# thegedge/StereoReconstruction

Measured on AMD Instinct MI355X. Metric: Mdisparity-hypotheses/s (WxHxD), higher is better.
Workload: dtype f64; 1 GPU; C3: synthetic rectified 1920x1080 pair, 256 depth levels, GeodesicWeight r=5; TwoView WTA both directions + cross-check; one pair per GPU; width=1920, height=1080, depth_levels=256, window_radius=5, weights=geodesic, pairs_per_gpu=1, pair_seed_rank0=1592590339, pair_seed_of_rank_r=seed + 0x10000*r, parallelism=single GPU

## Files before the change

include/stereo_recon_hip.h:

```cpp
#ifndef STEREO_RECON_HIP_H
#define STEREO_RECON_HIP_H

#include <stdint.h>
#include <stddef.h>

#ifdef __cplusplus
extern "C" {
#endif

#define SRH_ABI_VERSION 5

enum {
	SRH_OK = 0,
	SRH_E_INVALID = -1,
	SRH_E_DEVICE = -2,
	SRH_E_NO_DEVICE = -3,
	SRH_E_CANCELLED = -4,
	SRH_E_UNSUPPORTED = -5
};

enum { SRH_WEIGHT_ADAPTIVE = 0, SRH_WEIGHT_GEODESIC = 1 };
enum { SRH_MAX_VIEWS = 64 };
#define SRH_MAX_VIEW_DIM 32767

// ... 34 lines not shown

typedef struct srh_stats {
	int64_t n_pixels;
	int64_t n_eval;
	int64_t n_eval_device;
	int32_t used_dense_path;
	int32_t used_fused_kernel;
	int32_t used_strip_kernel;
	int32_t band_retries;
	int64_t n_certified;
	int64_t n_flagged;
	int64_t band_budget_bytes;
	int64_t mvs_waves_staged, mvs_waves_listed;
	int64_t scan_tiles_template, scan_tiles_walked;
	int64_t scan_tiles_bound;
} srh_stats;

typedef struct srh_context srh_context;

typedef void (*srh_progress_fn)(int step, const char *stage, void *user);

int         srh_abi_version(void);
const char *srh_build_id(void);
const char *srh_last_error(void);
int         srh_device_count(int *count);
int         srh_hw_queues_requested(void);

void srh_params_twoview_defaults(srh_params *p);
void srh_params_mvs_defaults(srh_params *p);
int  srh_camera_from_krt(const double K[9], const double R[9], const double t[3],
// ... 260 lines not shown
```

stereoreconstruction_amd/capi.py:

```python
import ctypes as C
import os

import numpy as np

_HERE = os.path.dirname(os.path.abspath(__file__))
LIB_PATH = os.environ.get("SRH_LIBRARY") or os.path.join(_HERE, "libstereo_recon_hip.so")

SRH_OK = 0
SRH_E_INVALID, SRH_E_DEVICE, SRH_E_NO_DEVICE, SRH_E_CANCELLED, SRH_E_UNSUPPORTED = -1, -2, -3, -4, -5
WEIGHT_ADAPTIVE, WEIGHT_GEODESIC = 0, 1
MAX_VIEWS = 64
MAX_VIEW_DIM = 32767

c_double_p = C.POINTER(C.c_double)
c_int32_p = C.POINTER(C.c_int32)
c_uint8_p = C.POINTER(C.c_uint8)


class Camera(C.Structure):
    _fields_ = [
        ("K", C.c_double * 9), ("Kinv", C.c_double * 9), ("R", C.c_double * 9), ("Rinv", C.c_double * 9),
        ("t", C.c_double * 3), ("C", C.c_double * 3),
        ("dist", C.c_double * 5),
        ("is_distorted", C.c_int32), ("is_refractive", C.c_int32),
# ... 47 lines not shown


LABEL_PIXEL_NONE = -2147483648

ARITH_EXACT, ARITH_FMA, ARITH_F32, ARITH_CERTIFIED = 0, 1, 2, 3
ARITH_DEFAULT = ARITH_CERTIFIED


class Stats(C.Structure):
    _fields_ = [("n_pixels", C.c_int64), ("n_eval", C.c_int64), ("n_eval_device", C.c_int64),
                ("used_dense_path", C.c_int32), ("used_fused_kernel", C.c_int32),
                ("used_strip_kernel", C.c_int32), ("band_retries", C.c_int32),
                ("n_certified", C.c_int64), ("n_flagged", C.c_int64), ("band_budget_bytes", C.c_int64),
                ("mvs_waves_staged", C.c_int64), ("mvs_waves_listed", C.c_int64),
                ("scan_tiles_template", C.c_int64), ("scan_tiles_walked", C.c_int64),
                ("scan_tiles_bound", C.c_int64)]


class FilterInfo(C.Structure):
    _fields_ = [("holes", C.c_int64), ("gap_filled", C.c_int64), ("median_filled", C.c_int64), ("replayed", C.c_int64)]


FILTER_GAPS, FILTER_MEDIAN = 1, 2


class FuseParams(C.Structure):
    _fields_ = [("dist_threshold", C.c_double), ("normal_depth_gap", C.c_double), ("min_views", C.c_int32), ("flags", C.c_int32)]


class FuseInfo(C.Structure):
    _fields_ = [("n_points", C.c_int64), ("n_candidates", C.c_int64), ("n_claimed", C.c_int64),
# ... 949 lines not shown
        sl = np.ascontiguousarray(view_slots, dtype=np.int32)
        _check(lib().srh_comm_allgather_views(self._h, sl.ctypes.data_as(c_int32_p), len(sl)))

    def comm_destroy(self):
        _check(lib().srh_comm_destroy(self._h))

    def stats(self):
        s = Stats()
        _check(lib().srh_get_stats(self._h, C.byref(s)))
        return dict(n_pixels=s.n_pixels, n_eval=s.n_eval, n_eval_device=s.n_eval_device,
                    used_dense_path=bool(s.used_dense_path), used_fused_kernel=bool(s.used_fused_kernel),
                    used_strip_kernel=bool(s.used_strip_kernel), band_retries=s.band_retries,
                    n_certified=s.n_certified, n_flagged=s.n_flagged, band_budget_bytes=s.band_budget_bytes,
                    mvs_waves_staged=s.mvs_waves_staged, mvs_waves_listed=s.mvs_waves_listed,
                    scan_tiles_template=s.scan_tiles_template, scan_tiles_walked=s.scan_tiles_walked,
                    scan_tiles_bound=s.scan_tiles_bound)

    def profile_enable(self, on=True):
        _check(lib().srh_profile_enable(self._h, int(on)))

    def profile_reset(self):
        _check(lib().srh_profile_reset(self._h))

    def profile(self):
        buf = C.create_string_buffer(1 << 16)
        _check(lib().srh_profile_dump(self._h, buf, len(buf)))
        out = {}
        for line in buf.value.decode().splitlines():
            name, ms, n = line.split()
            out[name] = (float(ms), int(n))
        return out
# ... 1 lines not shown
```

stereoreconstruction_amd/csrc/srh_api.hip:

```cpp
#include "srh_internal.hpp"
#include "srh_subpixel.hpp"
#include "srh_mvs_subpixel.hpp"
#include "srh_geom.hpp"
#include "srh_walk.hpp"
#include "srh_speckle.hpp"
#include "srh_rectify.hpp"

#include <algorithm>
#include <cassert>
#include <cstdarg>
#include <cstdio>
#include <cstdlib>
#include <cstring>
#include <map>
#include <mutex>
#include <string>
#include <utility>
#include <limits>
#include <vector>

using namespace srh;

static thread_local char g_err[512] = "";

// ... 213 lines not shown
#ifndef SRH_MVS_SLOTS
#define SRH_MVS_SLOTS 2
#endif
struct MvsSlot {
	hipStream_t stream = nullptr;
	hipEvent_t ev = nullptr, done = nullptr;
	int *h_maxc = nullptr;
	bool own_buffers = false;
	Scratch mem;
	bool pending = false;
	int view = -1, nneigh = 0, y0 = 0, y1 = 0, cmax = 0;
	int32_t neigh[SRH_MAX_NEIGH] = {0};
	srh_params p;
};

struct srh_context {
	int device = 0;
	hipStream_t own_stream = nullptr;
	hipStream_t stream = nullptr;
	ViewHost views[SRH_MAX_VIEWS];
	DevBuf<ViewDev> d_views;
	DevBuf<int32_t> d_slots;
	int32_t slots_host[SRH_MAX_VIEWS] = {0}; int slots_n = 0;
	Scratch mem;
	hipStream_t mrf_stream[SRH_MAX_VIEWS] = { nullptr };
	hipEvent_t views_go = nullptr;
	void *mrf_host = nullptr;
	DevBuf<double> mrf_peaks;
	DevBuf<double> mvs_subpx;
	int mvs_subpx_search = 0;
	double *mvsgm_host = nullptr;
	LabelStage mrf   { "single-view MRF", "MRF", 'K' };
	LabelStage mvsgm { "single-view SGM", "SGM", 'K' };
	LabelStage tvmrf { "TwoView MRF", "TwoView MRF", 'L' };
	LabelStage tvsgm { "TwoView SGM", "TwoView SGM", 'L' };
	LabelStage *const label_stages[4] = { &mrf, &mvsgm, &tvmrf, &tvsgm };
	int geodma = 1;
	int tscan_bound = 1;
	int tscan = 1;
	int strip = 1;
	int num_cus = 256;
	bool force_walk = false;
	int list_count_pass = 0;
	int list_cmax_hint = 0;
	int list_smax_hint = 0;
	int mvs_cmax_hint = 0;
	hipStream_t side_stream = nullptr;
	hipEvent_t side_go = nullptr, side_done = nullptr;
	hipEvent_t side_tpl = nullptr;
	int mvs_async = 1;
	MvsSlot mvs_slot[SRH_MVS_SLOTS];
	int mvs_turn = 0, mvs_last = -1;
	int mvs_staged = 1;
// ... 534 lines not shown
	if (!strcmp(name, "wta_outputs")) {
		if (value != 0 && value != SRH_WTA_WINNERS && value != (SRH_WTA_WINNERS | SRH_WTA_COSTS))
			return fail(SRH_E_INVALID, "wta_outputs must be 0, 1 (SRH_WTA_WINNERS) or 3 (SRH_WTA_WINNERS | SRH_WTA_COSTS): the costs are those of the kept winners");
		c->wta_outputs = (int)value; return SRH_OK;
	}
	if (!strcmp(name, "subpixel")) {
		if (value != 0 && value != 1) return fail(SRH_E_INVALID, "subpixel must be 0 or 1");
		c->subpixel = (int)value; return SRH_OK;
	}
	if (!strcmp(name, "mvs_subpixel_search")) {
		if (value != 0 && value != 1) return fail(SRH_E_INVALID, "mvs_subpixel_search must be 0 or 1");
		c->mvs_subpx_search = (int)value; return SRH_OK;
	}
	if (!strcmp(name, "tscan")) { c->tscan = value != 0; return SRH_OK; }
	if (!strcmp(name, "tscan_bound")) { c->tscan_bound = value != 0; return SRH_OK; }
	if (!strcmp(name, "geodma")) { c->geodma = value != 0; return SRH_OK; }
	if (!strcmp(name, "f32_form")) { c->f32_form = value != 0; return SRH_OK; }
	if (!strcmp(name, "rows_masked")) { c->rows_masked = (int)value; return SRH_OK; }
	if (!strcmp(name, "side_weights")) { c->side_weights = value != 0; return SRH_OK; }
	if (!strcmp(name, "debug_mvs_cmax_hint")) { c->mvs_cmax_hint = value > 0 ? (int)((value + 7) & ~7L) : 0; return SRH_OK; }
#ifdef SRH_EXPERIMENT
	if (!strcmp(name, "exp_repeat")) { exp_set((int)value, -1); return SRH_OK; }
	if (!strcmp(name, "exp_lds_pad")) { exp_set(-1, (int)value); return SRH_OK; }
	if (!strcmp(name, "exp_scan_mode")) { exp_set_scan((int)value); return SRH_OK; }
	if (!strcmp(name, "exp_walk_mode")) { exp_set_walk((int)value); return SRH_OK; }
	if (!strcmp(name, "exp_rows_mode")) { exp_set_rows((int)value); return SRH_OK; }
#endif
	return fail(SRH_E_INVALID, "unknown option '%s'", name);
}

// ... 406 lines not shown
	HIP_TRY(hipMemcpyAsync(host, dev, bytes, hipMemcpyDeviceToHost, st));
	HIP_TRY(hipStreamSynchronize(st));
	return SRH_OK;
}

static int fetch_counters(srh_context *c, const Lane &lane, int used_dense) {
	Counters h;
	int rc;
	if ((rc = read_back(lane.stream, &h, lane.mem->cnt, sizeof(h)))) return rc;
	c->stats.n_pixels = (int64_t)h.n_pixels;
	c->stats.n_eval = (int64_t)h.n_eval;
	c->stats.n_eval_device = (int64_t)h.n_eval_device;
	c->stats.scan_tiles_template = (int64_t)h.scan_tiles_template;
	c->stats.scan_tiles_walked = (int64_t)h.scan_tiles_walked;
	c->stats.scan_tiles_bound = (int64_t)h.scan_tiles_bound;
	c->stats.mvs_waves_staged = (int64_t)h.mvs_waves_staged;
	c->stats.mvs_waves_listed = (int64_t)h.mvs_waves_listed;
	c->stats.used_dense_path = used_dense;
	c->stats.used_fused_kernel = c->last_fused ? 1 : 0;
#ifdef SRH_PROFILE_PHASES
	{
		unsigned long long g[8];
		geodesic_phases_fetch(g);
		if (g[7])
			fprintf(stderr, "[srh prof] geodesic kernel: %llu waves, cycles per wave: staging %.0f  sweeps %.0f  exp %.0f  rows out %.0f  pconst: first sweep %.0f  second sweep %.0f  rest %.0f\n",
			        g[7], (double)g[0]/g[7], (double)g[1]/g[7], (double)g[2]/g[7], (double)g[4]/g[7], (double)g[5]/g[7], (double)g[6]/g[7], (double)g[3]/g[7]);
	}
	if (h.dbg_redo[4])
		fprintf(stderr, "[srh prof] redo kernel: %llu pixels, cycles per pixel (first wave): projections + mask %.0f  walk %.0f  wait for the columns %.0f  "
		        "running minimum %.0f | second wave: columns %.0f\n", h.dbg_redo[4], (double)h.dbg_redo[0]/h.dbg_redo[4], (double)h.dbg_redo[1]/h.dbg_redo[4],
// ... 694 lines not shown
}

int TvPass::run_dense(TvDense &D) const {
	int rc;
	if ((rc = dense_prepare(D))) return rc;
	const int cost_arith = c->arith == 3 ? (D.cert ? (c->cert_form == 1 ? 5 : 3) : 0) : c->arith;
	for (int by = y0; by < y1; by += (int)D.rows) {
		if (cancelled(c)) return fail(SRH_E_CANCELLED, "cancelled");
		const int nr = std::min((int)D.rows, y1 - by);
		if ((rc = dense_band_inputs(D, by, nr, cost_arith))) return rc;
		if (D.cert) HIP_TRY(hipMemsetAsync(lane.mem->band.cflag, 0, sizeof(uint32_t), lane.stream));
		if ((rc = dense_cost_pass(D, by, nr, cost_arith, false))) return rc;
		if (D.tpl_wait) { HIP_TRY(hipStreamWaitEvent(lane.stream, c->side_tpl, 0)); D.tpl_wait = false; }
		{ Scope s(c, lane.stream, "twoview_scan_kernel");
		  launch_twoview_scan(lane.stream, c->d_views, ref, oth, W, *p, by, nr, lane.mem->band.tnum, lane.mem->band.cost, D.cstride, lane.mem->cnt, lane.mem->band.prange,
		                      D.cert ? lane.mem->band.cflag : nullptr, -1, D.cert && D.strip ? lane.mem->band.pconst : nullptr, D.tscan ? lane.mem->band.stpl : nullptr, lane.mem->band.tileflag, c->num_cus, wout, c->tscan_bound); }
		if (D.cert) {
			const int cap = redo_capacity((size_t)nr*W);
			if (twoview_redo_takes(*p, D.cstride)) {
				Scope s(c, lane.stream, "twoview_redo_kernel");
				launch_twoview_redo(lane.stream, c->d_views, ref, oth, W, *p, by, lane.mem->band.tnum, lane.mem->band.wbuf, D.strip, c->views[ref].tvp,
				                    c->views[oth].tvp, lane.mem->band.cost, D.cstride, lane.mem->band.prange, lane.mem->band.cflag, cap, lane.mem->cnt, wout);
			} else {
				{ Scope s(c, lane.stream, "twoview_refill_kernel");
				  launch_twoview_refill(lane.stream, W, *p, by, lane.mem->band.prange, lane.mem->band.cflag, cap, lane.mem->band.wbuf, D.strip, c->views[ref].tvp,
				                        c->views[oth].tvp, lane.mem->band.cost, D.cstride, lane.mem->cnt); }
				Scope s(c, lane.stream, "twoview_rescan_kernel");
				launch_twoview_scan(lane.stream, c->d_views, ref, oth, W, *p, by, nr, lane.mem->band.tnum, lane.mem->band.cost, D.cstride, lane.mem->cnt, lane.mem->band.prange,
				                    lane.mem->band.cflag, cap, nullptr, nullptr, nullptr, c->num_cus, wout);
			}
		}
// ... 2130 lines not shown
```

stereoreconstruction_amd/csrc/srh_dense.hip:

```cpp
#include "srh_internal.hpp"
#include "srh_geom.hpp"
#include "srh_walk.hpp"
#include "srh_block.hpp"

#include <algorithm>
#include <type_traits>
#include <utility>

namespace srh {

__device__ __forceinline__ double color_dist_u(uint32_t a, uint32_t b) {
	const double dr = (double)((int)(a & 255u) - (int)(b & 255u));
	const double dg = (double)((int)((a >> 8) & 255u) - (int)((b >> 8) & 255u));
	const double db = (double)((int)((a >> 16) & 255u) - (int)((b >> 16) & 255u));
	return sqrt(dr*dr + dg*dg + db*db);
}

__global__ void edge_planes_kernel(const uint32_t *__restrict__ rgba, int W, int H, double *__restrict__ edges)
{
	const size_t n = (size_t)W*H;
	const double inf = __builtin_inf();
	for (size_t i = (size_t)blockIdx.x*blockDim.x + threadIdx.x; i < n; i += (size_t)gridDim.x*blockDim.x) {
		const int x = (int)(i % (size_t)W), y = (int)(i / (size_t)W);
		const uint32_t c = rgba[i];
// ... 1551 lines not shown
			x1 = x2;
		}
	}
	return good;
}

#define TS_U 8
template <bool CERT, bool WTA>
__device__ __forceinline__
bool twoview_tscan_tile(const int bid, const ViewDev *__restrict__ views, int ref, int oth, const srh_params &P,
                        int y0, int nrows, const double *__restrict__ tnum,
                        const double *__restrict__ cost, int cstride,
                        Counters *__restrict__ cnt, const PixRange *__restrict__ prange,
                        uint32_t *__restrict__ cflag, const CertBound &cb, const double *__restrict__ pexact,
                        const ScanTemplate *__restrict__ tpl, unsigned char *smask, unsigned &n_eval_acc, unsigned &n_pix_acc, unsigned &n_flag_acc,
                        int32_t *__restrict__ wout, const int use_bound, bool &by_bound)
{
	const ViewDev &L = views[ref];
	const ViewDev &Rv = views[oth];
	const int W = L.w, OW = Rv.w, OH = Rv.h;
	const int tiles_per_row = (W + SC_TW - 1)/SC_TW;
	const int tid = threadIdx.x;
	const int trow = bid / tiles_per_row;
	const int xt = (bid % tiles_per_row)*SC_TW, x = xt + tid;
	const int y = y0 + trow;
	const int D = P.num_depth_levels;
#ifdef SRH_EXPERIMENT
	if (g_exp_scan_mode == 6) return true;
#endif
	const int nS = tpl->nS, smin = tpl->smin, smax = tpl->smax;
	const bool active = x < W && L.mask[(size_t)y*W + x] == 1;
	bool good = true;
	bool verify = true;
#ifdef SRH_EXPERIMENT
	verify = g_exp_scan_mode != 3 && g_exp_scan_mode != 5;
#endif
	by_bound = false;
	if (verify) {
		bool bpass = false;
		if (active) {
			const Ray ray = cam_unproject(L.cam, (x + 0.5) / P.image_scale, (y + 0.5) / P.image_scale);
			const TsPixel pp = ts_pixel_setup(ray, L.cam, Rv.cam, P.image_scale, tpl->tabs, tpl->tmin, tpl->tmax, y);
			good = good && pp.ok;
			if (use_bound && good) bpass = ts_pixel_passes(pp, tpl->m, ts_pixel_E(pp, tpl->m, P.image_scale, (double)(x - tpl->x0)));
		}
		if (__any(active && !good)) return false;
		if (!use_bound || __any(active && !bpass)) {
			if (active) {
				const Ray ray = cam_unproject(L.cam, (x + 0.5) / P.image_scale, (y + 0.5) / P.image_scale);
				const TsPixel pp = ts_pixel_setup(ray, L.cam, Rv.cam, P.image_scale, tpl->tabs, tpl->tmin, tpl->tmax, y);
				good = tscan_verify_labels(pp.fp, pp.nd, pp.eU, pp.dyU, P.image_scale, x, D, tpl, tnum);
			}
// ... 4 lines not shown
	if (active) {
		const PixRange pr = prange[(size_t)trow*W + x];
		lo = pr.lo;
		const int hi = pr.hi;
		int wlo = x + smin, whi = x + smax;
		if (whi == -1) whi = 0;
		if (wlo < 0) wlo = 0;
		if (whi > OW - 1) whi = OW - 1;
		good = true;
		if (nS > 0 && whi >= wlo) good = lo <= wlo && hi >= whi;
		if (y < 0 || y >= OH) good = false;
	}
	if (__any(active && !good)) return false;

	const int mbase = xt + smin, mlen = nS > 0 ? SC_TW + (smax - smin) + 1 : 0;
	for (int k = tid; k < mlen; k += SC_TW) {
		const int tx = mbase + k;
		smask[k] = ((unsigned)tx < (unsigned)OW) ? Rv.mask[(size_t)y*OW + tx] : (unsigned char)0;
	}
	__syncthreads();

	unsigned n_eval = 0, n_flag = 0;
	double depth = __builtin_nan("");
	int owin = -1, orun = -1;
	if (active) {
		n_pix_acc += 1;
		const double *crow = cost + ((size_t)trow*((W + DC_TP - 1)/DC_TP) + (x/DC_TP))*(size_t)cstride*DC_TP + (x % DC_TP);
		WtaState<int, WTA> st(-1);
		bool px_sure = false;
		if (CERT && pexact) { const double *pc = pexact + ((size_t)trow*W + x)*SRH_PC; px_sure = cert_pixel_exact(cb, pc[2], pc[3]); }
		const int xm = tid - smin;
		const int xlo = x - lo;
		int nSe = nS;
#ifdef SRH_EXPERIMENT
		if (g_exp_scan_mode == 4 || g_exp_scan_mode == 5) nSe = 0;
#endif
		auto lookups = [&](auto left_c) {
			constexpr bool LEFT = decltype(left_c)::value;
			const int32_t *seq = LEFT ? tpl->S : tpl->F;
			const int nE = nSe == 0 ? 0 : (LEFT ? nS : tpl->nF);
			for (int j0 = 0; j0 < nE; j0 += TS_U) {
				int sv[TS_U], kk[TS_U], mu[TS_U];
				unsigned char mb[TS_U];
				double c[TS_U];
				{
					const int4 sa = reinterpret_cast<const int4 *>(&seq[j0])[0], sb = reinterpret_cast<const int4 *>(&seq[j0])[1];
					sv[0] = sa.x; sv[1] = sa.y; sv[2] = sa.z; sv[3] = sa.w; sv[4] = sb.x; sv[5] = sb.y; sv[6] = sb.z; sv[7] = sb.w;
				}
#pragma unroll
				for (int u = 0; u < TS_U; ++u) {
					int s;
// ... 4 lines not shown
					} else {
						s = (sv[u] << 8) >> 8;
						mu[u] = sv[u] >> 24;
					}
					sv[u] = s;
					mb[u] = smask[xm + s];
				}
#pragma unroll
				for (int u = 0; u < TS_U; ++u) {
					const bool white = j0 + u < nE && mb[u] == 1;
					n_eval += white ? (unsigned)mu[u] : 0u;
					kk[u] = white ? xlo + sv[u] : -1;
					c[u] = crow[(unsigned)(white ? kk[u] : 0)*(unsigned)DC_TP];
				}
#pragma unroll
				for (int u = 0; u < TS_U; ++u) {
					const bool on = kk[u] >= 0;
					const double cv = c[u];
					const double t = on ? cv + P.wta_margin : __builtin_inf();
					if (CERT) {
						if (__any(on && cert_step_near(t, st.minCost, cb))) {
							if (on && cert_step_doubt(cv, t, st.minCost, kk[u] == st.win, px_sure, cb, P.max_color_diff)) n_flag = 1;
						}
					}
					st.take_sum(t, cv, kk[u]);
				}
			}
		};
		if (xt + smin < 0 || !(P.wta_margin >= 0.0)) lookups(std::true_type()); else lookups(std::false_type());
		if (st.win >= 0) depth = candidate_depth(L.cam, Rv.cam, P, cam_unproject(L.cam, (x + 0.5) / P.image_scale, (y + 0.5) / P.image_scale), lo + st.win, y);
		if (st.rejected(P.second_best_factor)) depth = __builtin_inf();
		if (CERT && st.win >= 0 && cert_ratio_doubt(st.minCost, st.secondBest, P.second_best_factor, px_sure, cb, P.max_color_diff)) n_flag = 1;
		if (CERT && n_flag) cflag[1 + atomicAdd(&cflag[0], 1u)] = (uint32_t)((size_t)trow*W + x);
		if (WTA) { owin = st.win >= 0 ? lo + st.win : -1; orun = st.run >= 0 ? lo + st.run : -1; }
	}
	if (x < W) L.depth[(size_t)y*W + x] = depth;
	if (WTA && x < W) wta_store(wout, (size_t)W*L.h, (size_t)y*W + x, owin, owin >= 0 ? y : -1, orun, orun >= 0 ? y : -1);
	n_eval_acc += n_eval; n_flag_acc += n_flag;
	return true;
}

template <bool CERT, bool WTA>
__global__ __launch_bounds__(SC_TW, (CERT && WTA) ? 6 : 7)
void twoview_tscan_kernel(const ViewDev *__restrict__ views, int ref, int oth, srh_params P,
                          int y0, int nrows, const double *__restrict__ tnum,
                          const double *__restrict__ cost, int cstride,
                          Counters *__restrict__ cnt, const PixRange *__restrict__ prange,
                          uint32_t *__restrict__ cflag, CertBound cb, const double *__restrict__ pexact,
                          const ScanTemplate *__restrict__ tpl, uint32_t *__restrict__ tilelist, int32_t *__restrict__ wout, int use_bound)
{
	__shared__ unsigned char smask[SC_TW + TS_MAXSPAN + 16];
	const int W = views[ref].w;
	const int ntiles = ((W + SC_TW - 1)/SC_TW)*nrows;
	const int tid = threadIdx.x;
	const bool tok = tpl->ok != 0;
	unsigned n_eval = 0, n_pix = 0, n_flag = 0, n_tpl = 0, n_walk = 0, n_bound = 0;
	for (int bid = blockIdx.x; bid < ntiles; bid += gridDim.x) {
		bool by_bound = false;
		const bool done = tok && twoview_tscan_tile<CERT, WTA>(bid, views, ref, oth, P, y0, nrows, tnum, cost, cstride, cnt, prange, cflag, cb, pexact,
		                                                      tpl, smask, n_eval, n_pix, n_flag, wout, use_bound, by_bound);
		if (!done) { if (tid == 0) tilelist[1 + atomicAdd(&tilelist[0], 1u)] = (uint32_t)bid; ++n_walk; } else { ++n_tpl; n_bound += by_bound ? 1u : 0u; }
		__syncthreads();
	}
	if (!cnt) return;
	n_eval = wave_sum_u32(n_eval); n_pix = wave_sum_u32(n_pix); n_flag = wave_sum_u32(n_flag);
	if (tid == 0) {
		if (n_eval) atomicAdd(&cnt->n_eval, (unsigned long long)n_eval);
		if (n_pix) atomicAdd(&cnt->n_pixels, (unsigned long long)n_pix);
		if (CERT && n_pix) atomicAdd(&cnt->n_certified, (unsigned long long)n_pix);
		if (CERT && n_flag) atomicAdd(&cnt->n_flagged, (unsigned long long)n_flag);
		if (n_tpl) atomicAdd(&cnt->scan_tiles_template, (unsigned long long)n_tpl);
		if (n_walk) atomicAdd(&cnt->scan_tiles_walked, (unsigned long long)n_walk);
		if (n_bound) atomicAdd(&cnt->scan_tiles_bound, (unsigned long long)n_bound);
	}
}

#define RSW_MAXD 1024
#define RSW_MAXC 6144
#define RD_THREADS 512
#define RD_GRID 512
template <int R, bool WTA>
__global__ __launch_bounds__(RD_THREADS)
void twoview_redo_kernel(const ViewDev *__restrict__ views, int ref, int oth, srh_params P, int y0,
                         const double *__restrict__ tnum, const double *__restrict__ wbuf, int wimg,
                         const double *__restrict__ ref_tvp, const double *__restrict__ oth_tvp,
                         double *__restrict__ cost, int cstride,
                         const PixRange *__restrict__ prange, const uint32_t *__restrict__ cflag, int cap,
                         Counters *__restrict__ cnt, int32_t *__restrict__ wout)
{
	const ViewDev &L = views[ref];
	const ViewDev &Rv = views[oth];
	const int W = L.w, OW = Rv.w, OH = Rv.h;
	const int tid = threadIdx.x;
	__shared__ double sx[RSW_MAXD], sy[RSW_MAXD];
	__shared__ unsigned short scol[RSW_MAXC];
	__shared__ double srow[4096];
	__shared__ unsigned char smask[4096 + 64];
	__shared__ int s_n;
	const uint32_t nflag = cflag[0];
	if (blockIdx.x == 0 && tid == 0 && nflag > (uint32_t)cap) atomicAdd(&cnt->cert_overflow, 1ull);
	unsigned n_cols = 0;
#ifdef SRH_PROFILE_PHASES
	unsigned long long rph[6] = {0, 0, 0, 0, 0, 0}, rt = __builtin_readcyclecounter();
#define RD_STAMP(k) do { const unsigned long long tn_ = __builtin_readcyclecounter(); rph[k] += tn_ - rt; rt = tn_; } while (0)
#else
#define RD_STAMP(k)
#endif
	for (uint32_t f = blockIdx.x; f < nflag && f < (uint32_t)cap; f += gridDim.x) {
		const uint32_t q = cflag[1 + f];
		const int x = (int)(q % (uint32_t)W), trow = (int)(q / (uint32_t)W), y = y0 + trow;
		const PixRange pr = prange[q];
		const int lo = pr.lo, hi = pr.hi;
// ... 3 lines not shown
		const bool walk = !(fabs(nd) < 1e-10);
		if (walk) {
			const SharedDivisor nd_sd = shared_divisor(nd);
			for (int d = tid; d < P.num_depth_levels; d += RD_THREADS) {
				double x2, y2;
				const bool ok = pinhole_project_label_sd(ray, nd_sd, tnum[d], Rv.cam, P.image_scale, x2, y2);
				sx[d] = ok ? x2 : __builtin_nan("");
				sy[d] = ok ? y2 : 0.0;
			}
		}
		const int span = hi >= lo ? hi - lo + 1 : 0;
		for (int k = tid; k < span && k < 4096; k += RD_THREADS) smask[k] = (y >= 0 && y < OH) ? Rv.mask[(size_t)y*OW + lo + k] : 0;
		__syncthreads();
		RD_STAMP(0);
		double *crow = cost + ((size_t)trow*((W + DC_TP - 1)/DC_TP) + (x/DC_TP))*(size_t)cstride*DC_TP + (x % DC_TP);
		if (tid == 0) {
			int n = 0;
			bool over = false;
			if (walk) {
				double x1 = __builtin_nan(""), y1 = __builtin_nan("");
				for (int d = 0; d < P.num_depth_levels && !over; ++d) {
					const double x2 = sx[d], y2 = sy[d];
					if (isnan_d(x2)) continue;
					if (isnan_d(x1)) { x1 = x2; y1 = y2; continue; }
					const double dx = x2 - x1, dy = y2 - y1;
					if (!(dx*dx + dy*dy >= 1)) continue;
					const int ix0 = trunc_sat(x1), iy0 = trunc_sat(y1), ix1 = trunc_sat(x2), iy1 = trunc_sat(y2);
					const int a = ix0 < ix1 ? ix0 : ix1, b = ix0 < ix1 ? ix1 : ix0;
					if (iy0 == y && iy1 == y && a >= lo && b <= hi) {
						for (int tx = a; tx <= b; ++tx) {
							const int k = tx - lo;
							const bool white = k < 4096 ? (smask[k] == 1) : (Rv.mask[(size_t)y*OW + tx] == 1);
							if (white) { if (n < RSW_MAXC) scol[n] = (unsigned short)k; else over = true; ++n; }
						}
// ... 2 lines not shown
						lw.begin(ix0, iy0, ix1, iy1, OW, OH);
						while (lw.has_next()) {
							int tx, ty;
							lw.current(tx, ty);
							if (tx >= 0 && ty >= 0 && tx < OW && ty < OH && Rv.mask[(size_t)ty*OW + tx] == 1 &&
							    ty == y && tx >= lo && tx <= hi) {
								if (n < RSW_MAXC) scol[n] = (unsigned short)(tx - lo); else over = true;
								++n;
							}
							lw.next();
						}
					}
					x1 = x2; y1 = y2;
				}
			}
			if (over) { atomicAdd(&cnt->cert_overflow, 1ull); n = RSW_MAXC; }
			s_n = n;
		} else if (tid >= 64) {
			const int SP = padded_stride(W);
			const WindowAt wa = window_at<R>(wbuf, wimg, W, trow, x);
			const double *lp = ref_tvp + (size_t)(y + SRH_PADY - R)*SP + (x + SRH_PADL - R);
			for (int c = lo + (tid - 64); c <= hi; c += RD_THREADS - 64) {
				const double *rp = oth_tvp + (size_t)(y + SRH_PADY - R)*SP + (c + SRH_PADL - R);
				const double cv = window_exact_cost<R>(wa.wq, wa.wrow, wa.wcol, lp, rp, SP, SP, P);
				crow[(size_t)(c - lo)*DC_TP] = cv;
				if (c - lo < 4096) srow[c - lo] = cv;
				++n_cols;
			}
		}
		RD_STAMP(1);
		__syncthreads();
		RD_STAMP(2);
		if (tid == 0) {
// ... 37 lines not shown
	if (P.window_radius == 5) { if (wout) SRH_REDO(5, true); else SRH_REDO(5, false); }
	else                      { if (wout) SRH_REDO(2, true); else SRH_REDO(2, false); }
#undef SRH_REDO
	return true;
}

void launch_scan_template(hipStream_t st, const ViewDev *views, int ref, int oth, const srh_params &P, int y0, int nrows,
                          const double *tnum, void *tpl)
{
	hipLaunchKernelGGL(twoview_template_kernel, dim3(1), dim3(256), 0, st, views, ref, oth, P, y0, nrows, tnum, (ScanTemplate *)tpl);
}

void launch_twoview_scan(hipStream_t st, const ViewDev *views, int ref, int oth, int width, const srh_params &P,
                         int y0, int nrows, const double *tnum, const double *cost, int cstride,
                         Counters *cnt, const PixRange *prange, uint32_t *cflag, int nlist, const double *pexact,
                         const void *tpl, uint32_t *tilelist, int num_cus, int32_t *wout, int tscan_bound)
{
	const int tiles = (width + SC_TW - 1)/SC_TW;
	const CertBound cb = cert_bound(P);
	const ScanTemplate *tp = (const ScanTemplate *)tpl;
	if (!tp) tilelist = nullptr;
	const unsigned pgrid = (unsigned)std::min<long long>((long long)tiles*nrows, (long long)num_cus*4*8);
	const unsigned wgrid = tp ? (unsigned)std::min<long long>((long long)tiles*nrows, (long long)num_cus*4*4) : (unsigned)(tiles*nrows);
	if (tp) (void)hipMemsetAsync(tilelist, 0, sizeof(uint32_t), st);
#define SRH_TSCAN(C_, W_, FLAG_, PEX_)                                                                         \
	hipLaunchKernelGGL((twoview_tscan_kernel<C_, W_>), dim3(pgrid), dim3(SC_TW), 0, st,                        \
	                   views, ref, oth, P, y0, nrows, tnum, cost, cstride, cnt, prange, FLAG_, cb, PEX_, tp, tilelist, wout, tscan_bound)
#define SRH_SCAN(C_, L_, W_, GRID_, FLAG_, NL_, PEX_, TL_)                                                     \
	hipLaunchKernelGGL((twoview_scan_kernel<C_, L_, W_>), dim3(GRID_), dim3(SC_TW), 0, st,                     \
	                   views, ref, oth, P, y0, nrows, tnum, cost, cstride, cnt, prange, FLAG_, NL_, cb, PEX_, TL_, wout)
	if (!cflag) {
		if (tp) { if (wout) SRH_TSCAN(false, true, nullptr, nullptr); else SRH_TSCAN(false, false, nullptr, nullptr); }
		if (wout) SRH_SCAN(false, false, true, wgrid, nullptr, 0, nullptr, tilelist);
		else      SRH_SCAN(false, false, false, wgrid, nullptr, 0, nullptr, tilelist);
	} else if (nlist < 0) {
		if (tp) { if (wout) SRH_TSCAN(true, true, cflag, pexact); else SRH_TSCAN(true, false, cflag, pexact); }
		if (wout) SRH_SCAN(true, false, true, wgrid, cflag, 0, pexact, tilelist);
		else      SRH_SCAN(true, false, false, wgrid, cflag, 0, pexact, tilelist);
	} else if (nlist > 0) {
		const unsigned lgrid = (unsigned)((nlist + SC_TW - 1)/SC_TW);
		if (wout) SRH_SCAN(false, true, true, lgrid, cflag, nlist, nullptr, nullptr);
		else      SRH_SCAN(false, true, false, lgrid, cflag, nlist, nullptr, nullptr);
// ... 7 lines not shown
```

stereoreconstruction_amd/csrc/srh_internal.hpp:

```cpp
#pragma once

#include <hip/hip_runtime.h>
#include <stdint.h>

#include "stereo_recon_hip.h"
#include "srh_wta.hpp"
#include "srh_stripframe.hpp"

namespace srh {

struct ViewDev {
	int32_t w, h;
	const uint32_t *rgba;
	const uint8_t  *mask;
	const double   *gray;
	const double   *gray_tv;
	double         *depth;
	srh_camera      cam;
	const uint64_t *census;
};

#define SRH_WTILE 32
__host__ __device__ inline size_t wbuf_doubles(int W, int nrows, int T) {
	return (size_t)nrows*((W + SRH_WTILE - 1)/SRH_WTILE)*SRH_WTILE*T;
// ... 24 lines not shown
void launch_twoview_winner_costs(hipStream_t st, const ViewDev *views, int ref, int oth, int width, const srh_params &P, int kind,
                                 int y0, int nrows, const double *wbuf, bool wimg, const int32_t *wout,
                                 double *min_cost, double *second_cost);

struct Counters {
	unsigned long long n_pixels;
	unsigned long long n_eval;
	unsigned long long n_eval_device;
	unsigned long long not_row_aligned;
	unsigned long long n_listed, n_slots;
	unsigned long long strip_overflow;
	unsigned long long n_certified, n_flagged;
	unsigned long long cert_overflow;
	unsigned long long scan_tiles_template, scan_tiles_walked;
	unsigned long long scan_tiles_bound;
	unsigned long long mvs_waves_staged, mvs_waves_listed;
	unsigned int strip_ticket, strip_ticket_border;
	unsigned long long dbg_cycles, dbg_blocks, dbg_total_cycles, dbg_waves;
	unsigned long long dbg_phase[8];
	unsigned long long dbg_wave[64];
	unsigned long long dbg_redo[6];
};

#define SRH_MAX_NEIGH 8
struct NeighList { int32_t n[SRH_MAX_NEIGH]; };
inline NeighList make_neigh_list(const int32_t *neigh, int nneigh) {
	NeighList l;
	for (int i = 0; i < SRH_MAX_NEIGH; ++i) l.n[i] = (i < nneigh) ? neigh[i] : 0;
	return l;
}
// ... 31 lines not shown
void launch_label_plane_table(hipStream_t st, const ViewDev *views, int ref, const srh_params &P, bool mvs, double *tdist);
void launch_pinhole_label_table(hipStream_t st, const ViewDev *views, int ref, const srh_params &P, bool mvs, double *tnum);
bool launch_twoview_dense_cost_f32(hipStream_t st, const ViewDev *views, int ref, int oth, int width, const srh_params &P,
                                   int y0, int nrows, const double *wbuf, size_t wstride,
                                   const double *tnum, double *cost, int cstride, Counters *cnt, const double *pconst, int form = 0);
bool launch_twoview_dense_cost(hipStream_t st, const ViewDev *views, int ref, int oth, int width, const srh_params &P,
                               int y0, int nrows, const double *wbuf, size_t wstride,
                               const double *tnum, double *cost, int cstride, Counters *cnt, const double *pconst, int arith = 0,
                               const PixRange *prange = nullptr);
void launch_twoview_scan(hipStream_t st, const ViewDev *views, int ref, int oth, int width, const srh_params &P,
                         int y0, int nrows, const double *tnum, const double *cost, int cstride,
                         Counters *cnt, const PixRange *prange, uint32_t *cflag = nullptr, int nlist = -1,
                         const double *pexact = nullptr,
                         const void *tpl = nullptr, uint32_t *tilelist = nullptr,
                         int num_cus = 256, int32_t *wout = nullptr,
                         int tscan_bound = 1);
size_t scan_template_bytes();
void launch_scan_template(hipStream_t st, const ViewDev *views, int ref, int oth, const srh_params &P, int y0, int nrows,
                          const double *tnum, void *tpl);
bool launch_twoview_refill(hipStream_t st, int width, const srh_params &P, int y0, const PixRange *prange, const uint32_t *cflag, int cap,
                           const double *wbuf, bool wimg, const double *ref_tvp, const double *oth_tvp, double *cost, int cstride, Counters *cnt);
bool twoview_redo_takes(const srh_params &P, int cstride);
bool launch_twoview_redo(hipStream_t st, const ViewDev *views, int ref, int oth, int width, const srh_params &P, int y0,
                         const double *tnum, const double *wbuf, bool wimg, const double *ref_tvp, const double *oth_tvp,
                         double *cost, int cstride, const PixRange *prange, const uint32_t *cflag, int cap, Counters *cnt, int32_t *wout);
void launch_twoview_lazy_fill(hipStream_t st, const ViewDev *views, int ref, int oth, int width, const srh_params &P,
                              int y0, int nrows, const PixRange *prange, const uint32_t *filllist, const double *wbuf, size_t wstride,
                              const double *ref_tvp, const double *oth_tvp,
                              bool wimg,
                              int lanes, bool padded,
                              double *cost, int cstride, Counters *cnt);
// ... 213 lines not shown
```

stereoreconstruction_amd/csrc/srh_wta.hpp:

```cpp
#pragma once

#include <math.h>
#include <stdint.h>

#include "stereo_recon_hip.h"

#if defined(__HIPCC__)
#include <hip/hip_runtime.h>
#endif
#ifndef SRH_NHD
#if defined(__HIPCC__)
#define SRH_NHD __host__ __device__ __forceinline__
#else
#define SRH_NHD inline
#endif
#endif

namespace srh {

struct WtaXY {
	int x, y;
	SRH_NHD bool operator==(const WtaXY &o) const { return x == o.x && y == o.y; }
	SRH_NHD bool operator!=(const WtaXY &o) const { return !(*this == o); }
};
// ... 51 lines not shown
	c.ok = c.room > 0 && c.m_hi > P.max_color_diff && P.max_color_diff <= 1e5 && fabs(P.bad_ret) <= 1e5 &&
	       P.wta_margin >= 0 && P.wta_margin <= 1e5 && fabs(P.second_best_factor) <= 1e5 && weights_ok;
	return c;
}

SRH_NHD bool cert_sure(double x, double clamp, double m_hi) { return x == clamp || x > m_hi; }
SRH_NHD bool cert_pixel_exact(const CertBound &cb, double sum2, double all_taps_usable) {
	return !(all_taps_usable != 0.0) || !(cb.sigma3(sum2) < __builtin_inf());
}
SRH_NHD bool cert_step_near(double t, double minCost, const CertBound &cb) { return !(fabs(t - minCost) > 2.5*cb.e0); }
SRH_NHD bool cert_step_doubt(double cost, double t, double minCost, bool is_winner, bool px_sure, const CertBound &cb, double clamp) {
	return cert_step_near(t, minCost, cb) && !is_winner &&
	       !(cert_sure(cost, clamp, cb.m_hi) && cert_sure(minCost, clamp, cb.m_hi)) &&
	       !(px_sure && cost == cost);
}
SRH_NHD bool cert_ratio_doubt(double minCost, double secondBest, double factor, bool px_sure, const CertBound &cb, double clamp) {
	const double rhs = factor*secondBest;
	const double tol = __builtin_fma(fmin(fabs(rhs), 1e300), 1e-15, (1.0 + fabs(factor))*cb.e0);
	return !(fabs(minCost - rhs) > tol) && !px_sure &&
	       !(cert_sure(minCost, clamp, cb.m_hi) && cert_sure(secondBest, clamp, cb.m_hi));
}

}
```

Measured before the change: 49400 Mhyp/s.

## Add lean template scan path and wave-parallel segment walk in redo kernel

Adds an opt-in lean scan loop for tiles whose whole mask span is valid. It skips per-entry mask LDS reads and uses precomputed byte offsets, with the template entry count packed in the high byte. Separately, the cert redo kernel now builds the candidate column list with a full wavefront: a ballot-based prefix sum over the mask, parallel segment detection via readlane, and a shuffle scan. Before, one thread walked all depth levels. The walk falls back to the serial path when segments leave the row or exceed the span, and the change adds LDS use and stats counters.

```diff
diff --git a/include/stereo_recon_hip.h b/include/stereo_recon_hip.h
--- a/include/stereo_recon_hip.h
+++ b/include/stereo_recon_hip.h
@@ -72,6 +72,7 @@
 	int64_t mvs_waves_staged, mvs_waves_listed;
 	int64_t scan_tiles_template, scan_tiles_walked;
 	int64_t scan_tiles_bound;
+	int64_t scan_tiles_lean;
 } srh_stats;
 
 typedef struct srh_context srh_context;
diff --git a/profiles/tscan_isa_count.py b/profiles/tscan_isa_count.py
--- /dev/null
+++ b/profiles/tscan_isa_count.py
@@ -0,0 +1,59 @@
+#!/usr/bin/env python3
+import re
+import sys
+
+TS_U = 8
+text = open(sys.argv[1]).read().split("\n")
+res = {}
+if len(sys.argv) > 2:
+    cur = None
+    for ln in open(sys.argv[2]):
+        m = re.search(r"Function Name: (\S+)", ln)
+        if m:
+            cur = m.group(1)
+            res[cur] = {}
+        m = re.search(r"(TotalSGPRs|VGPRs|ScratchSize \[bytes/lane\]|Occupancy \[waves/SIMD\]): (\d+)", ln)
+        if m and cur:
+            res[cur][m.group(1).split(" ")[0]] = int(m.group(2))
+
+kernels = [i for i, ln in enumerate(text) if re.match(r"_ZN3srh20twoview_tscan_kernelILb[01]ELb[01]E.*:\s*(;.*)?$", ln)]
+for k0 in kernels:
+    name = text[k0].split(":")[0]
+    cert, wta = re.search(r"ILb([01])ELb([01])E", name).groups()
+    k1 = next(i for i in range(k0, len(text)) if text[i].strip().startswith("s_endpgm"))
+    body = text[k0:k1]
+    labels = {ln.split(":")[0]: i for i, ln in enumerate(body) if re.match(r"\.LBB\d+_\d+:", ln)}
+    r = res.get(name, {})
+    print("twoview_tscan_kernel<CERT=%s, WTA=%s>: VGPRs %s  SGPRs %s  scratch %s  waves/SIMD %s" % (
+        cert, wta, r.get("VGPRs", "?"), r.get("TotalSGPRs", "?"), r.get("ScratchSize", "?"), r.get("Occupancy", "?")))
+    loops = []
+    for i, ln in enumerate(body):
+        m = re.match(r"\s+s_cbranch_\w+\s+(\.LBB\d+_\d+)", ln)
+        if m and m.group(1) in labels and labels[m.group(1)] < i:
+            loops.append((labels[m.group(1)], i))
+    found = 0
+    for a, b in loops:
+        if any(a < a2 and b2 < b for a2, b2 in loops):
+            continue
+        lines = [ln for ln in body[a:b + 1] if re.match(r"\s+[a-z]", ln) and not ln.strip().startswith(";")]
+        ins = [ln.split()[0] for ln in lines]
+        loads = [x for x in ins if x == "global_load_dwordx2"]
+        if len(loads) != TS_U:
+            continue
+        found += 1
+        lds = sum(1 for x in ins if x.startswith("ds_read"))
+        kind = "lean" if lds == 0 else ("left" if sum(1 for x in ins if x in ("s_bitcmp1_b32", "s_bitcmp0_b32")) >= TS_U else "general")
+        n = lambda pred: sum(1 for x in ins if pred(x)) / TS_U
+        add_s = sum(1 for ln in lines if ln.split()[0] == "v_lshl_add_u64" and re.search(r", s\[\d+:\d+\]\s*$", ln))
+        mad64 = sum(1 for x in ins if x.startswith("v_mad_u64") or x.startswith("v_mad_i64"))
+        print("  %-8s %4d instructions per %d entries; per entry: valu %.1f  salu %.1f  loads %.1f  lds reads %.1f  v_readlane %.1f  "
+              "exec branches %.1f  scalar branches %.1f;  addresses: %d lane base + scalar pair, %d per-lane 64-bit multiply-adds" % (
+                  kind, len(ins), TS_U,
+                  n(lambda x: x.startswith("v_") and x not in ("v_readlane_b32", "v_writelane_b32")),
+                  n(lambda x: x.startswith("s_") and not x.startswith("s_cbranch") and not x.startswith("s_waitcnt") and not x.startswith("s_load")),
+                  n(lambda x: x.startswith("global_load") or x.startswith("s_load")), lds / TS_U,
+                  n(lambda x: x == "v_readlane_b32"),
+                  n(lambda x: x in ("s_cbranch_execz", "s_cbranch_execnz")),
+                  n(lambda x: x.startswith("s_cbranch") and x not in ("s_cbranch_execz", "s_cbranch_execnz")), add_s, mad64))
+    if not found:
+        print("  (the doubt blocks lie out of line and jump back into the loops: no loop body is one run of lines here; count by hand)")
diff --git a/stereoreconstruction_amd/capi.py b/stereoreconstruction_amd/capi.py
--- a/stereoreconstruction_amd/capi.py
+++ b/stereoreconstruction_amd/capi.py
@@ -85,7 +85,7 @@
                 ("n_certified", C.c_int64), ("n_flagged", C.c_int64), ("band_budget_bytes", C.c_int64),
                 ("mvs_waves_staged", C.c_int64), ("mvs_waves_listed", C.c_int64),
                 ("scan_tiles_template", C.c_int64), ("scan_tiles_walked", C.c_int64),
-                ("scan_tiles_bound", C.c_int64)]
+                ("scan_tiles_bound", C.c_int64), ("scan_tiles_lean", C.c_int64)]
 
 
 class FilterInfo(C.Structure):
@@ -1065,7 +1065,7 @@
                     n_certified=s.n_certified, n_flagged=s.n_flagged, band_budget_bytes=s.band_budget_bytes,
                     mvs_waves_staged=s.mvs_waves_staged, mvs_waves_listed=s.mvs_waves_listed,
                     scan_tiles_template=s.scan_tiles_template, scan_tiles_walked=s.scan_tiles_walked,
-                    scan_tiles_bound=s.scan_tiles_bound)
+                    scan_tiles_bound=s.scan_tiles_bound, scan_tiles_lean=s.scan_tiles_lean)
 
     def profile_enable(self, on=True):
         _check(lib().srh_profile_enable(self._h, int(on)))
diff --git a/stereoreconstruction_amd/csrc/srh_api.hip b/stereoreconstruction_amd/csrc/srh_api.hip
--- a/stereoreconstruction_amd/csrc/srh_api.hip
+++ b/stereoreconstruction_amd/csrc/srh_api.hip
@@ -251,6 +251,10 @@
 	srh_params p;
 };
 
+#ifndef SRH_TSCAN_LEAN_DEFAULT
+#define SRH_TSCAN_LEAN_DEFAULT 0
+#endif
+
 struct srh_context {
 	int device = 0;
 	hipStream_t own_stream = nullptr;
@@ -274,6 +278,7 @@
 	LabelStage *const label_stages[4] = { &mrf, &mvsgm, &tvmrf, &tvsgm };
 	int geodma = 1;
 	int tscan_bound = 1;
+	int tscan_lean = SRH_TSCAN_LEAN_DEFAULT;
 	int tscan = 1;
 	int strip = 1;
 	int num_cus = 256;
@@ -838,6 +843,7 @@
 	}
 	if (!strcmp(name, "tscan")) { c->tscan = value != 0; return SRH_OK; }
 	if (!strcmp(name, "tscan_bound")) { c->tscan_bound = value != 0; return SRH_OK; }
+	if (!strcmp(name, "tscan_lean")) { c->tscan_lean = value != 0; return SRH_OK; }
 	if (!strcmp(name, "geodma")) { c->geodma = value != 0; return SRH_OK; }
 	if (!strcmp(name, "f32_form")) { c->f32_form = value != 0; return SRH_OK; }
 	if (!strcmp(name, "rows_masked")) { c->rows_masked = (int)value; return SRH_OK; }
@@ -1274,6 +1280,7 @@
 	c->stats.scan_tiles_template = (int64_t)h.scan_tiles_template;
 	c->stats.scan_tiles_walked = (int64_t)h.scan_tiles_walked;
 	c->stats.scan_tiles_bound = (int64_t)h.scan_tiles_bound;
+	c->stats.scan_tiles_lean = (int64_t)h.scan_tiles_lean;
 	c->stats.mvs_waves_staged = (int64_t)h.mvs_waves_staged;
 	c->stats.mvs_waves_listed = (int64_t)h.mvs_waves_listed;
 	c->stats.used_dense_path = used_dense;
@@ -1998,7 +2005,7 @@
 		if (D.tpl_wait) { HIP_TRY(hipStreamWaitEvent(lane.stream, c->side_tpl, 0)); D.tpl_wait = false; }
 		{ Scope s(c, lane.stream, "twoview_scan_kernel");
 		  launch_twoview_scan(lane.stream, c->d_views, ref, oth, W, *p, by, nr, lane.mem->band.tnum, lane.mem->band.cost, D.cstride, lane.mem->cnt, lane.mem->band.prange,
-		                      D.cert ? lane.mem->band.cflag : nullptr, -1, D.cert && D.strip ? lane.mem->band.pconst : nullptr, D.tscan ? lane.mem->band.stpl : nullptr, lane.mem->band.tileflag, c->num_cus, wout, c->tscan_bound); }
+		                      D.cert ? lane.mem->band.cflag : nullptr, -1, D.cert && D.strip ? lane.mem->band.pconst : nullptr, D.tscan ? lane.mem->band.stpl : nullptr, lane.mem->band.tileflag, c->num_cus, wout, c->tscan_bound, c->tscan_lean); }
 		if (D.cert) {
 			const int cap = redo_capacity((size_t)nr*W);
 			if (twoview_redo_takes(*p, D.cstride)) {
diff --git a/stereoreconstruction_amd/csrc/srh_dense.hip b/stereoreconstruction_amd/csrc/srh_dense.hip
--- a/stereoreconstruction_amd/csrc/srh_dense.hip
+++ b/stereoreconstruction_amd/csrc/srh_dense.hip
@@ -1589,7 +1589,7 @@
                         Counters *__restrict__ cnt, const PixRange *__restrict__ prange,
                         uint32_t *__restrict__ cflag, const CertBound &cb, const double *__restrict__ pexact,
                         const ScanTemplate *__restrict__ tpl, unsigned char *smask, unsigned &n_eval_acc, unsigned &n_pix_acc, unsigned &n_flag_acc,
-                        int32_t *__restrict__ wout, const int use_bound, bool &by_bound)
+                        int32_t *__restrict__ wout, const int use_bound, bool &by_bound, const int use_lean, bool &by_lean)
 {
 	const ViewDev &L = views[ref];
 	const ViewDev &Rv = views[oth];
@@ -1611,6 +1611,7 @@
 	verify = g_exp_scan_mode != 3 && g_exp_scan_mode != 5;
 #endif
 	by_bound = false;
+	by_lean = false;
 	if (verify) {
 		bool bpass = false;
 		if (active) {
@@ -1645,11 +1646,16 @@
 	if (__any(active && !good)) return false;
 
 	const int mbase = xt + smin, mlen = nS > 0 ? SC_TW + (smax - smin) + 1 : 0;
+	bool mall = true;
 	for (int k = tid; k < mlen; k += SC_TW) {
 		const int tx = mbase + k;
-		smask[k] = ((unsigned)tx < (unsigned)OW) ? Rv.mask[(size_t)y*OW + tx] : (unsigned char)0;
+		const unsigned char mbyte = ((unsigned)tx < (unsigned)OW) ? Rv.mask[(size_t)y*OW + tx] : (unsigned char)0;
+		smask[k] = mbyte;
+		mall = mall && mbyte == 1;
 	}
 	__syncthreads();
+	const bool lean = use_lean && mlen > 0 && xt + smin >= 0 && P.wta_margin >= 0.0 && !__any(!mall);
+	by_lean = lean;
 
 	unsigned n_eval = 0, n_flag = 0;
 	double depth = __builtin_nan("");
@@ -1666,6 +1672,7 @@
 #ifdef SRH_EXPERIMENT
 		if (g_exp_scan_mode == 4 || g_exp_scan_mode == 5) nSe = 0;
 #endif
+		auto wave_any = [](bool b) { return __builtin_amdgcn_ballot_w64(b) != 0; };
 		auto lookups = [&](auto left_c) {
 			constexpr bool LEFT = decltype(left_c)::value;
 			const int32_t *seq = LEFT ? tpl->S : tpl->F;
@@ -1700,20 +1707,50 @@
 					c[u] = crow[(unsigned)(white ? kk[u] : 0)*(unsigned)DC_TP];
 				}
 #pragma unroll
+				for (int u = 0; u < TS_U; ++u)
+					scan_step<CERT>(st, n_flag, c[u], kk[u], kk[u] >= 0, P.wta_margin, px_sure, cb, P.max_color_diff, wave_any);
+			}
+		};
+		auto lookups_lean = [&]() {
+			const int32_t *seq = tpl->F;
+			const int nE = nSe == 0 ? 0 : tpl->nF;
+			const int TS_NONE = -0x7fffffff - 1;
+			static_assert(SC_TW % DC_TP == 0, "a tile starts on a cost-row group: x/DC_TP = xt/DC_TP + tid/DC_TP");
+			const double *tbase = cost + ((size_t)trow*((W + DC_TP - 1)/DC_TP) + (xt/DC_TP))*(size_t)cstride*DC_TP;
+			const unsigned voff = (unsigned)(((tid/DC_TP)*cstride + (xlo + smin))*DC_TP + (tid % DC_TP))*(unsigned)sizeof(double);
+			WtaState<int, WTA> ls(TS_NONE);
+			unsigned msum = 0;
+			double margin = P.wta_margin;
+			asm volatile("" : "+v"(margin));
+			auto group = [&](auto whole_c, const int j0) {
+				constexpr bool WHOLE = decltype(whole_c)::value;
+				int sv[TS_U];
+				double c[TS_U];
+				{
+					const int4 sa = reinterpret_cast<const int4 *>(&seq[j0])[0], sb = reinterpret_cast<const int4 *>(&seq[j0])[1];
+					sv[0] = sa.x; sv[1] = sa.y; sv[2] = sa.z; sv[3] = sa.w; sv[4] = sb.x; sv[5] = sb.y; sv[6] = sb.z; sv[7] = sb.w;
+				}
+#pragma unroll
 				for (int u = 0; u < TS_U; ++u) {
-					const bool on = kk[u] >= 0;
-					const double cv = c[u];
-					const double t = on ? cv + P.wta_margin : __builtin_inf();
-					if (CERT) {
-						if (__any(on && cert_step_near(t, st.minCost, cb))) {
-							if (on && cert_step_doubt(cv, t, st.minCost, kk[u] == st.win, px_sure, cb, P.max_color_diff)) n_flag = 1;
-						}
-					}
-					st.take_sum(t, cv, kk[u]);
+					msum += (unsigned)(sv[u] >> 24);
+					sv[u] = (sv[u] << 8) >> 8;
+					const double *sp = tbase + (size_t)(sv[u] - smin)*DC_TP;
+					c[u] = *reinterpret_cast<const double *>(reinterpret_cast<const char *>(sp) + voff);
 				}
-			}
+#pragma unroll
+				for (int u = 0; u < TS_U; ++u)
+					scan_step<CERT>(ls, n_flag, c[u], sv[u], WHOLE || j0 + u < nE, margin, px_sure, cb, P.max_color_diff, wave_any);
+			};
+			const int nW = nE & ~(TS_U - 1);
+			for (int j0 = 0; j0 < nW; j0 += TS_U) group(std::true_type(), j0);
+			if (nW < nE) group(std::false_type(), nW);
+			n_eval += msum;
+			st.minCost = ls.minCost; st.secondBest = ls.secondBest;
+			st.win = ls.win == TS_NONE ? -1 : xlo + ls.win;
+			if (WTA) st.run = ls.run == TS_NONE ? -1 : xlo + ls.run;
 		};
-		if (xt + smin < 0 || !(P.wta_margin >= 0.0)) lookups(std::true_type()); else lookups(std::false_type());
+		if (lean) lookups_lean();
+		else if (xt + smin < 0 || !(P.wta_margin >= 0.0)) lookups(std::true_type()); else lookups(std::false_type());
 		if (st.win >= 0) depth = candidate_depth(L.cam, Rv.cam, P, cam_unproject(L.cam, (x + 0.5) / P.image_scale, (y + 0.5) / P.image_scale), lo + st.win, y);
 		if (st.rejected(P.second_best_factor)) depth = __builtin_inf();
 		if (CERT && st.win >= 0 && cert_ratio_doubt(st.minCost, st.secondBest, P.second_best_factor, px_sure, cb, P.max_color_diff)) n_flag = 1;
@@ -1733,19 +1770,20 @@
                           const double *__restrict__ cost, int cstride,
                           Counters *__restrict__ cnt, const PixRange *__restrict__ prange,
                           uint32_t *__restrict__ cflag, CertBound cb, const double *__restrict__ pexact,
-                          const ScanTemplate *__restrict__ tpl, uint32_t *__restrict__ tilelist, int32_t *__restrict__ wout, int use_bound)
+                          const ScanTemplate *__restrict__ tpl, uint32_t *__restrict__ tilelist, int32_t *__restrict__ wout, int use_bound, int use_lean)
 {
 	__shared__ unsigned char smask[SC_TW + TS_MAXSPAN + 16];
 	const int W = views[ref].w;
 	const int ntiles = ((W + SC_TW - 1)/SC_TW)*nrows;
 	const int tid = threadIdx.x;
 	const bool tok = tpl->ok != 0;
-	unsigned n_eval = 0, n_pix = 0, n_flag = 0, n_tpl = 0, n_walk = 0, n_bound = 0;
+	unsigned n_eval = 0, n_pix = 0, n_flag = 0, n_tpl = 0, n_walk = 0, n_bound = 0, n_lean = 0;
 	for (int bid = blockIdx.x; bid < ntiles; bid += gridDim.x) {
-		bool by_bound = false;
+		bool by_bound = false, by_lean = false;
 		const bool done = tok && twoview_tscan_tile<CERT, WTA>(bid, views, ref, oth, P, y0, nrows, tnum, cost, cstride, cnt, prange, cflag, cb, pexact,
-		                                                      tpl, smask, n_eval, n_pix, n_flag, wout, use_bound, by_bound);
-		if (!done) { if (tid == 0) tilelist[1 + atomicAdd(&tilelist[0], 1u)] = (uint32_t)bid; ++n_walk; } else { ++n_tpl; n_bound += by_bound ? 1u : 0u; }
+		                                                      tpl, smask, n_eval, n_pix, n_flag, wout, use_bound, by_bound, use_lean, by_lean);
+		if (!done) { if (tid == 0) tilelist[1 + atomicAdd(&tilelist[0], 1u)] = (uint32_t)bid; ++n_walk; }
+		else { ++n_tpl; n_bound += by_bound ? 1u : 0u; n_lean += by_lean ? 1u : 0u; }
 		__syncthreads();
 	}
 	if (!cnt) return;
@@ -1758,9 +1796,13 @@
 		if (n_tpl) atomicAdd(&cnt->scan_tiles_template, (unsigned long long)n_tpl);
 		if (n_walk) atomicAdd(&cnt->scan_tiles_walked, (unsigned long long)n_walk);
 		if (n_bound) atomicAdd(&cnt->scan_tiles_bound, (unsigned long long)n_bound);
-	}
-}
-
+		if (n_lean) atomicAdd(&cnt->scan_tiles_lean, (unsigned long long)n_lean);
+	}
+}
+
+__device__ __forceinline__ double lane_read_f64(double v, int lane) {
+	return __hiloint2double(__builtin_amdgcn_readlane(__double2hiint(v), lane), __builtin_amdgcn_readlane(__double2loint(v), lane));
+}
 #define RSW_MAXD 1024
 #define RSW_MAXC 6144
 #define RD_THREADS 512
@@ -1782,6 +1824,7 @@
 	__shared__ unsigned short scol[RSW_MAXC];
 	__shared__ double srow[4096];
 	__shared__ unsigned char smask[4096 + 64];
+	__shared__ unsigned short spre[4096 + 8];
 	__shared__ int s_n;
 	const uint32_t nflag = cflag[0];
 	if (blockIdx.x == 0 && tid == 0 && nflag > (uint32_t)cap) atomicAdd(&cnt->cert_overflow, 1ull);
@@ -1815,10 +1858,61 @@
 		__syncthreads();
 		RD_STAMP(0);
 		double *crow = cost + ((size_t)trow*((W + DC_TP - 1)/DC_TP) + (x/DC_TP))*(size_t)cstride*DC_TP + (x % DC_TP);
-		if (tid == 0) {
+		if (tid < 64) {
 			int n = 0;
 			bool over = false;
-			if (walk) {
+			bool on_wave = walk && span <= 4096;
+			if (on_wave) {
+				unsigned whites = 0;
+				for (int k0 = 0; k0 < span; k0 += 64) {
+					const int k = k0 + tid;
+					const unsigned long long wb = __builtin_amdgcn_ballot_w64(k < span && smask[k] == 1);
+					if (k < span) spre[k] = (unsigned short)(whites + __builtin_amdgcn_mbcnt_hi((unsigned)(wb >> 32), __builtin_amdgcn_mbcnt_lo((unsigned)wb, 0u)));
+					whites += (unsigned)__popcll(wb);
+				}
+				if (tid == 0) spre[span] = (unsigned short)whites;
+				__builtin_amdgcn_fence(__ATOMIC_RELEASE, "workgroup");
+				__builtin_amdgcn_wave_barrier();
+				__builtin_amdgcn_fence(__ATOMIC_ACQUIRE, "workgroup");
+				const int D = P.num_depth_levels;
+				double x1 = __builtin_nan(""), y1 = __builtin_nan("");
+				for (int r0 = 0; r0 < D; r0 += 64) {
+					const int d = r0 + tid;
+					const double lx = d < D ? sx[d] : __builtin_nan(""), ly = d < D ? sy[d] : 0.0;
+					bool seg = false;
+					double px = 0.0, py = 0.0;
+					const int nj = D - r0 < 64 ? D - r0 : 64;
+					for (int j = 0; j < nj; ++j) {
+						const double x2 = lane_read_f64(lx, j), y2 = lane_read_f64(ly, j);
+						if (isnan_d(x2)) continue;
+						if (isnan_d(x1)) { x1 = x2; y1 = y2; continue; }
+						const double dx = x2 - x1, dy = y2 - y1;
+						if (!(dx*dx + dy*dy >= 1)) continue;
+						if (tid == j) { seg = true; px = x1; py = y1; }
+						x1 = x2; y1 = y2;
+					}
+					int a = 0, b = -1, nw = 0;
+					bool fits = true;
+					if (seg) {
+						const int ix0 = trunc_sat(px), iy0 = trunc_sat(py), ix1 = trunc_sat(lx), iy1 = trunc_sat(ly);
+						a = ix0 < ix1 ? ix0 : ix1; b = ix0 < ix1 ? ix1 : ix0;
+						fits = iy0 == y && iy1 == y && a >= lo && b <= hi;
+						if (fits) nw = (int)spre[b - lo + 1] - (int)spre[a - lo];
+					}
+					if (__builtin_amdgcn_ballot_w64(!fits) != 0) { on_wave = false; break; }
+					int incl = nw;
+					for (int o = 1; o < 64; o <<= 1) { const int up = __shfl_up(incl, o, 64); if (tid >= o) incl += up; }
+					int at = n + incl - nw;
+					for (int tx = a; tx <= b; ++tx) {
+						const int k = tx - lo;
+						if (smask[k] == 1) { if (at < RSW_MAXC) scol[at] = (unsigned short)k; ++at; }
+					}
+					n += __builtin_amdgcn_readlane(incl, 63);
+				}
+				over = on_wave && n > RSW_MAXC;
+			}
+			if (!on_wave && tid == 0 && walk) {
+				n = 0;
 				double x1 = __builtin_nan(""), y1 = __builtin_nan("");
 				for (int d = 0; d < P.num_depth_levels && !over; ++d) {
 					const double x2 = sx[d], y2 = sy[d];
@@ -1851,9 +1945,11 @@
 					x1 = x2; y1 = y2;
 				}
 			}
-			if (over) { atomicAdd(&cnt->cert_overflow, 1ull); n = RSW_MAXC; }
-			s_n = n;
-		} else if (tid >= 64) {
+			if (tid == 0) {
+				if (over) { atomicAdd(&cnt->cert_overflow, 1ull); n = RSW_MAXC; }
+				s_n = n;
+			}
+		} else {
 			const int SP = padded_stride(W);
 			const WindowAt wa = window_at<R>(wbuf, wimg, W, trow, x);
 			const double *lp = ref_tvp + (size_t)(y + SRH_PADY - R)*SP + (x + SRH_PADL - R);
@@ -1921,7 +2017,7 @@
 void launch_twoview_scan(hipStream_t st, const ViewDev *views, int ref, int oth, int width, const srh_params &P,
                          int y0, int nrows, const double *tnum, const double *cost, int cstride,
                          Counters *cnt, const PixRange *prange, uint32_t *cflag, int nlist, const double *pexact,
-                         const void *tpl, uint32_t *tilelist, int num_cus, int32_t *wout, int tscan_bound)
+                         const void *tpl, uint32_t *tilelist, int num_cus, int32_t *wout, int tscan_bound, int tscan_lean)
 {
 	const int tiles = (width + SC_TW - 1)/SC_TW;
 	const CertBound cb = cert_bound(P);
@@ -1932,7 +2028,7 @@
 	if (tp) (void)hipMemsetAsync(tilelist, 0, sizeof(uint32_t), st);
 #define SRH_TSCAN(C_, W_, FLAG_, PEX_)                                                                         \
 	hipLaunchKernelGGL((twoview_tscan_kernel<C_, W_>), dim3(pgrid), dim3(SC_TW), 0, st,                        \
-	                   views, ref, oth, P, y0, nrows, tnum, cost, cstride, cnt, prange, FLAG_, cb, PEX_, tp, tilelist, wout, tscan_bound)
+	                   views, ref, oth, P, y0, nrows, tnum, cost, cstride, cnt, prange, FLAG_, cb, PEX_, tp, tilelist, wout, tscan_bound, tscan_lean)
 #define SRH_SCAN(C_, L_, W_, GRID_, FLAG_, NL_, PEX_, TL_)                                                     \
 	hipLaunchKernelGGL((twoview_scan_kernel<C_, L_, W_>), dim3(GRID_), dim3(SC_TW), 0, st,                     \
 	                   views, ref, oth, P, y0, nrows, tnum, cost, cstride, cnt, prange, FLAG_, NL_, cb, PEX_, TL_, wout)
diff --git a/stereoreconstruction_amd/csrc/srh_internal.hpp b/stereoreconstruction_amd/csrc/srh_internal.hpp
--- a/stereoreconstruction_amd/csrc/srh_internal.hpp
+++ b/stereoreconstruction_amd/csrc/srh_internal.hpp
@@ -62,6 +62,7 @@
 	unsigned long long cert_overflow;
 	unsigned long long scan_tiles_template, scan_tiles_walked;
 	unsigned long long scan_tiles_bound;
+	unsigned long long scan_tiles_lean;
 	unsigned long long mvs_waves_staged, mvs_waves_listed;
 	unsigned int strip_ticket, strip_ticket_border;
 	unsigned long long dbg_cycles, dbg_blocks, dbg_total_cycles, dbg_waves;
@@ -123,7 +124,8 @@
                          const double *pexact = nullptr,
                          const void *tpl = nullptr, uint32_t *tilelist = nullptr,
                          int num_cus = 256, int32_t *wout = nullptr,
-                         int tscan_bound = 1);
+                         int tscan_bound = 1,
+                         int tscan_lean = 0);
 size_t scan_template_bytes();
 void launch_scan_template(hipStream_t st, const ViewDev *views, int ref, int oth, const srh_params &P, int y0, int nrows,
                           const double *tnum, void *tpl);
diff --git a/stereoreconstruction_amd/csrc/srh_wta.hpp b/stereoreconstruction_amd/csrc/srh_wta.hpp
--- a/stereoreconstruction_amd/csrc/srh_wta.hpp
+++ b/stereoreconstruction_amd/csrc/srh_wta.hpp
@@ -89,6 +89,18 @@
 	       !(cert_sure(cost, clamp, cb.m_hi) && cert_sure(minCost, clamp, cb.m_hi)) &&
 	       !(px_sure && cost == cost);
 }
+template <bool CERT, class Id, bool WTA, class Any>
+SRH_NHD void scan_step(WtaState<Id, WTA> &st, unsigned &flag, double cost, Id id, bool on, double margin, bool px_sure,
+                       const CertBound &cb, double clamp, Any any) {
+	const double t = on ? cost + margin : __builtin_inf();
+	if (CERT) {
+		if (any(on && cert_step_near(t, st.minCost, cb))) {
+			if (on && cert_step_doubt(cost, t, st.minCost, id == st.win, px_sure, cb, clamp)) flag = 1;
+		}
+	}
+	st.take_sum(t, cost, id);
+}
+
 SRH_NHD bool cert_ratio_doubt(double minCost, double secondBest, double factor, bool px_sure, const CertBound &cb, double clamp) {
 	const double rhs = factor*secondBest;
 	const double tol = __builtin_fma(fmin(fabs(rhs), 1e300), 1e-15, (1.0 + fabs(factor))*cb.e0);
```

Measured after the change: 49460 Mhyp/s, median of 6. Within noise of the previous version (+0.1%).
